# nyasyamorina/font-renderer

Measured on AMD Instinct MI355X. Metric: Mpixel/s AA glyph coverage, higher is better.
Workload: dtype f32

## Files before the change

font-renderer_amd/csrc/fr_c4.hpp:

```cpp
#pragma once
#include "fr_records.hpp"
#include "fr_wave.hpp"

namespace fr {

#ifndef FR_C4_WAVES
#define FR_C4_WAVES 4
#endif
#ifndef FR_C4_OCC
#define FR_C4_OCC 4
#endif
#ifndef FR_C4_PCAP
#define FR_C4_PCAP 448
#endif
#ifndef FR_C4_OCC_SMALL
#define FR_C4_OCC_SMALL 6
#endif
#ifndef FR_DYN_BANDS
#define FR_DYN_BANDS 1
#endif
#ifndef FR_W1_OCC_SMALL
#define FR_W1_OCC_SMALL 6
#endif
enum { C4_WAVES = FR_C4_WAVES, C4_PCAP = FR_C4_PCAP };
// ... 7 lines not shown
    const uint2 a = reinterpret_cast<const uint2 *>(p)[0], b = reinterpret_cast<const uint2 *>(p)[1];
    return make_uint4(a.x, a.y, b.x, b.y);
}
template <uint32_t LSTRIDE>
__device__ __forceinline__ void c4_st16(uint16_t *p, uint4 v)
{
    if ((LSTRIDE * 2) % 16 == 0) { *reinterpret_cast<uint4 *>(p) = v; return; }
    reinterpret_cast<uint2 *>(p)[0] = make_uint2(v.x, v.y);
    reinterpret_cast<uint2 *>(p)[1] = make_uint2(v.z, v.w);
}

struct __attribute__((aligned(8))) Rec40 {
    float a;
    float b;
    float c1, c2;
    float ax, bx, p0x;
    float rden;
    float sgn;
    uint32_t fr;
};

__device__ __forceinline__ uint32_t c4_sel(unsigned long long m, uint32_t if_set, uint32_t if_clear)
{
    uint32_t r;
    asm("v_cndmask_b32_e64 %0, %1, %2, %3" : "=v"(r) : "v"(if_clear), "v"(if_set), "s"(m));
    return r;
}
__device__ __forceinline__ float c4_self(unsigned long long m, float if_set, float if_clear)
{
    return __builtin_bit_cast(float, c4_sel(m, __builtin_bit_cast(uint32_t, if_set), __builtin_bit_cast(uint32_t, if_clear)));
}
__device__ __forceinline__ void c4_store16(void *dst, uint4 v)
{
    typedef uint32_t u32x4 __attribute__((ext_vector_type(4)));
    typedef u32x4 u32x4_u __attribute__((aligned(4)));
    u32x4 w = {v.x, v.y, v.z, v.w};
    __builtin_nontemporal_store(w, reinterpret_cast<u32x4_u *>(dst));
}

template <int FILL = 0>
__device__ __forceinline__ Rec40 c4_make_rec40(const Rec &r, uint32_t ra, uint32_t re)
{
    Rec40 m;
    const bool lin = (int32_t)r.flags < 0;
    m.a = lin ? r.c1 : r.a;
    m.b = r.b; m.c1 = lin ? 0.0f : r.c1; m.c2 = r.c2;
    m.ax = r.ax; m.bx = r.bx; m.p0x = r.p0x; m.rden = r.rden;
    m.sgn = r.sqsign ? -1.0f : 1.0f;
    const uint32_t cb = (lin || FILL) ? (r.flags & 2u) : 2u, zb = (lin || FILL) ? cb : 0u;
    m.fr = ra | (re << 12) | (cb << 24) | (zb << 26) | (lin ? 0x80000000u : 0u);
    return m;
}

template <uint32_t RCAP, int N, uint32_t NCOL, int FILL>
__device__ __forceinline__ uint32_t c4_setup_small(const RenderArgs &A, const Job &job, uint32_t seg0, uint32_t nseg, uint32_t x0s,
                                                   int phase, float *s_cxp, Rec40 *s_rec, uint32_t *s_wcnt, uint32_t *s_tmp, const float *cyt = nullptr)
{
    const uint32_t tid = threadIdx.x, lane = tid & 63u, wave = tid >> 6;
    const uint32_t Hs = job.h * (uint32_t)N;
    RowGeom geo;
    geo.max_y = job.max_y; geo.scale = job.scale; geo.rows = Hs; geo.n = N; geo.phase = phase; geo.cyt = cyt;
    const bool have = lane < 2u * nseg;
    Rec r;
    RowGuess g;
    Piece pc;
    g.empty = true; g.ra = 1u; g.re = 0u;
    uint32_t cls = 3u;
    if (have) {
        record_prep<FILL>(A.seg_pts + 6u * (size_t)(seg0 + (lane >> 1)), lane & 1u, geo, r, g, &pc);
        if (!g.empty) {
            const uint32_t row = (wave == 0u) ? g.ra - 1u : (wave == 1u) ? g.ra : (wave == 2u) ? g.re - 1u : g.re;
            if (row < Hs && (wave != 2u || g.re > g.ra)) cls = (uint32_t)row_class<FILL>(r, pc, geo.cy(row));
        }
    }
    s_tmp[tid] = cls;
    const int32_t min_xs = job.min_x + (int32_t)x0s;
    for (uint32_t j = tid; j < NCOL; j += 256u)
        s_cxp[1u + j] = ((float)(min_xs + (int32_t)(j / (uint32_t)N)) + sub_off((int)(j % (uint32_t)N), N, phase)) / job.scale;
    if (tid == 2) s_cxp[0] = -__builtin_inff();
    if (tid == 3) s_cxp[1u + NCOL] = __builtin_inff();
    __syncthreads();
    if (wave == 0u) {
        Rec40 mine;
        mine.fr = 0u;
        bool live = false;
        if (have) {
            uint32_t ra = g.ra, re = g.re;
            if (!g.empty) {
                const uint32_t c0 = s_tmp[lane], c1 = s_tmp[64u + lane], c2 = s_tmp[128u + lane], c3 = s_tmp[192u + lane];
                const bool ok = (c0 >= 2u) && (c1 <= 1u || c1 == 3u) && re >= ra && (c2 >= 1u) && (c3 == 0u || c3 == 3u);
                if (!ok) record_settle<FILL>(r, geo, ra, re, &pc);
            }
            live = ra < re;
            mine = c4_make_rec40<FILL>(r, ra, re);
        }
        const bool linr = live && (int32_t)mine.fr < 0;
        const unsigned long long lm = __ballot(live && !linr), ll = __ballot(linr), below = (1ull << lane) - 1ull;
        const uint32_t n_quad = (uint32_t)__popcll(lm);
        uint32_t pos = RCAP;
        if ((lm >> lane) & 1ull) pos = (uint32_t)__popcll(lm & below);
        if ((ll >> lane) & 1ull) pos = n_quad + (uint32_t)__popcll(ll & below);
        if (pos < RCAP) s_rec[pos] = mine;
        if (lane == 0u) s_wcnt[0] = min(n_quad + (uint32_t)__popcll(ll), RCAP);
    }
    __syncthreads();
    return s_wcnt[0];
}

template <uint32_t RCAP, int N, uint32_t NCOL, int FILL>
__device__ __forceinline__ uint32_t c4_setup_mid(const RenderArgs &A, const Job &job, uint32_t seg0, uint32_t nseg, uint32_t x0s,
                                                 int phase, float *s_cxp, Rec40 *s_rec, uint32_t *s_wcnt, uint32_t *s_tmp, const float *cyt = nullptr)
{
    const uint32_t tid = threadIdx.x, lane = tid & 63u, wave = tid >> 6;
    const uint32_t c = tid & 127u, h = tid >> 7;
    const uint32_t Hs = job.h * (uint32_t)N;
    RowGeom geo;
    geo.max_y = job.max_y; geo.scale = job.scale; geo.rows = Hs; geo.n = N; geo.phase = phase; geo.cyt = cyt;
    const bool have = c < 2u * nseg;
    Rec r;
    RowGuess g;
    Piece pc;
    g.empty = true; g.ra = 1u; g.re = 0u;
    uint32_t cls0 = 3u, cls1 = 3u;
    if (have) {
        record_prep<FILL>(A.seg_pts + 6u * (size_t)(seg0 + (c >> 1)), c & 1u, geo, r, g, &pc);
        if (!g.empty) {
            const uint32_t end = h ? g.re : g.ra;
            if (end - 1u < Hs && (h == 0u || g.re > g.ra)) cls0 = (uint32_t)row_class<FILL>(r, pc, geo.cy(end - 1u));
            if (end < Hs) cls1 = (uint32_t)row_class<FILL>(r, pc, geo.cy(end));
        }
    }
    s_tmp[tid] = cls0 | (cls1 << 8);
    const int32_t min_xs = job.min_x + (int32_t)x0s;
    for (uint32_t j = tid; j < NCOL; j += 256u)
        s_cxp[1u + j] = ((float)(min_xs + (int32_t)(j / (uint32_t)N)) + sub_off((int)(j % (uint32_t)N), N, phase)) / job.scale;
    if (tid == 2) s_cxp[0] = -__builtin_inff();
    if (tid == 3) s_cxp[1u + NCOL] = __builtin_inff();
    __syncthreads();
    Rec40 mine;
    mine.fr = 0u;
    bool live = false;
    if (h == 0u && have) {
        uint32_t ra = g.ra, re = g.re;
        if (!g.empty) {
            const uint32_t up = s_tmp[c], dn = s_tmp[128u + c];
            const uint32_t c0 = up & 0xffu, c1 = up >> 8, c2 = dn & 0xffu, c3 = dn >> 8;
            const bool ok = (c0 >= 2u) && (c1 <= 1u || c1 == 3u) && re >= ra && (c2 >= 1u) && (c3 == 0u || c3 == 3u);
            if (!ok) record_settle<FILL>(r, geo, ra, re, &pc);
        }
        live = ra < re;
        mine = c4_make_rec40<FILL>(r, ra, re);
    }
    const bool linr = live && (int32_t)mine.fr < 0;
    const unsigned long long lm = __ballot(live && !linr), ll = __ballot(linr), below = (1ull << lane) - 1ull;
    if (lane == 0u && wave < 2u) { s_wcnt[wave] = (uint32_t)__popcll(lm); s_wcnt[2u + wave] = (uint32_t)__popcll(ll); }
    __syncthreads();
    const uint32_t q0 = s_wcnt[0], q1 = s_wcnt[1], l0 = s_wcnt[2], l1 = s_wcnt[3];
    const uint32_t n_quad = q0 + q1;
    uint32_t pos = RCAP;
    if ((lm >> lane) & 1ull) pos = (wave ? q0 : 0u) + (uint32_t)__popcll(lm & below);
    if ((ll >> lane) & 1ull) pos = n_quad + (wave ? l0 : 0u) + (uint32_t)__popcll(ll & below);
    if (wave < 2u && pos < RCAP) s_rec[pos] = mine;
    __syncthreads();
    return min(n_quad + l0 + l1, RCAP);
}

template <uint32_t NW, uint32_t RCAP, int N, uint32_t NCOL, int FILL = 0>
__device__ __forceinline__ uint32_t c4_setup(const RenderArgs &A, const Job &job, uint32_t seg0, uint32_t nseg, uint32_t x0s,
                                             int phase, float *s_cxp, Rec40 *s_rec, uint32_t *s_wcnt, uint32_t *s_tmp, const float *cyt = nullptr)
{
    if (NW == 4u && 2u * nseg <= 64u)
        return c4_setup_small<RCAP, N, NCOL, FILL>(A, job, seg0, nseg, x0s, phase, s_cxp, s_rec, s_wcnt, s_tmp, cyt);
    if (NW == 4u && 2u * nseg <= 128u)
        return c4_setup_mid<RCAP, N, NCOL, FILL>(A, job, seg0, nseg, x0s, phase, s_cxp, s_rec, s_wcnt, s_tmp, cyt);
    const uint32_t tid = threadIdx.x, lane = tid & 63u, wave = tid >> 6;
    const uint32_t Hs = job.h * (uint32_t)N;
    constexpr uint32_t CPT = (RCAP >= 1024u ? 1536u : (RCAP >= 512u ? 768u : 512u)) / (64u * NW);
    s_wcnt = s_tmp;
    Rec40 mine[CPT];
    unsigned long long lm[CPT], ll[CPT];
#pragma unroll
    for (uint32_t it = 0; it < CPT; ++it) {
        const uint32_t c = tid + it * 64u * NW;
        bool live = false;
        lm[it] = 0ull; ll[it] = 0ull;
        mine[it].fr = 0u;
        if (it > 0 && it * 64u * NW >= 2u * nseg) continue;
        if (c < 2u * nseg) {
            Rec r;
            RowGeom geo;
            geo.max_y = job.max_y; geo.scale = job.scale; geo.rows = Hs; geo.n = N; geo.phase = phase; geo.cyt = cyt;
            build_record_rows<FILL>(A.seg_pts + 6u * (size_t)(seg0 + (c >> 1)), c & 1u, geo, r);
            const uint32_t ra = __builtin_bit_cast(uint32_t, r.lo), re = __builtin_bit_cast(uint32_t, r.hi);
            live = ra < re;
            mine[it] = c4_make_rec40<FILL>(r, ra, re);
        }
        const bool linr = live && (int32_t)mine[it].fr < 0;
        lm[it] = __ballot(live && !linr);
        ll[it] = __ballot(linr);
        if (lane == 0) { s_wcnt[it * NW + wave] = (uint32_t)__popcll(lm[it]); s_wcnt[CPT * NW + it * NW + wave] = (uint32_t)__popcll(ll[it]); }
    }
    const int32_t min_xs = job.min_x + (int32_t)x0s;
    for (uint32_t j = tid; j < NCOL; j += 64u * NW)
        s_cxp[1u + j] = ((float)(min_xs + (int32_t)(j / (uint32_t)N)) + sub_off((int)(j % (uint32_t)N), N, phase)) / job.scale;
    if (tid == 2) s_cxp[0] = -__builtin_inff();
    if (tid == 3) s_cxp[1u + NCOL] = __builtin_inff();
    __syncthreads();
    uint32_t rec_cnt = 0;
    {
        uint32_t base_q[CPT], base_l[CPT], n_quad = 0;
#pragma unroll
        for (uint32_t it = 0; it < CPT; ++it) base_q[it] = base_l[it] = 0;
#pragma unroll
        for (uint32_t q = 0; q < CPT * NW; ++q) {
            if (q >= NW && q / NW * 64u * NW >= 2u * nseg) continue;
            const uint32_t cq = s_wcnt[q], cl = s_wcnt[CPT * NW + q];
#pragma unroll
            for (uint32_t it = 0; it < CPT; ++it) {
                base_q[it] += (q < it * NW + wave) ? cq : 0u;
                base_l[it] += (q < it * NW + wave) ? cl : 0u;
            }
            n_quad += cq;
            rec_cnt += cq + cl;
        }
#pragma unroll
        for (uint32_t it = 0; it < CPT; ++it) {
            const unsigned long long below = (1ull << lane) - 1ull;
            uint32_t pos = RCAP;
            if ((lm[it] >> lane) & 1ull) pos = base_q[it] + (uint32_t)__popcll(lm[it] & below);
            if ((ll[it] >> lane) & 1ull) pos = n_quad + base_l[it] + (uint32_t)__popcll(ll[it] & below);
            if (pos < RCAP) s_rec[pos] = mine[it];
        }
    }
    rec_cnt = min(rec_cnt, RCAP);
    __syncthreads();
    return rec_cnt;
}

}
```

font-renderer_amd/csrc/fr_cov4_kernel.inc:

```
    using L = C4Lds<WLOG, RPL, NS, CAP>;
    constexpr uint32_t LSTRIDE = L::LSTRIDE;
    static_assert(NS == 4 || NS == 2, "samples per axis");
    constexpr uint32_t RCAP = L::RCAP;
    constexpr uint32_t NW = C4_WAVES;
    constexpr uint32_t SW = 16u << WLOG;
    constexpr uint32_t NCOL = SW * (uint32_t)NS;
    constexpr uint32_t NWIN = 1u << WLOG;
    constexpr uint32_t PRB = L::PRB;
    constexpr int LN = (NS == 4) ? 2 : 1;
    constexpr bool SPLIT = RPL >= 8 && CAP == 32;
    extern __shared__ __align__(16) unsigned char smem[];

    const uint32_t tid = threadIdx.x, lane = tid & 63u;
    const uint32_t wave = (uint32_t)__builtin_amdgcn_readfirstlane((int)(tid >> 6));
    uint32_t bid = blockIdx.x, strip = 0, bgrp = 0;
    if (A.strips != 1u) { strip = bid % A.strips; bid /= A.strips; }
    if (A.band_groups != 1u) { bgrp = bid % A.band_groups; bid /= A.band_groups; }
    const uint32_t jidx = bid;
    C4_ABL_LAUNCH_ONLY();
    const Job job = A.jobs[jidx];
    const uint32_t x0s = strip * SW;
    const uint32_t band_first = bgrp * A.bands_per_wg;
    if (band_first * PRB >= job.h || x0s >= job.w) return;
    const uint32_t band_end = min(band_first + A.bands_per_wg, (job.h + PRB - 1u) / PRB);
    const uint32_t wlim = min(SW, job.w - x0s);
    const int phase = A.phase_center;
    const uint32_t seg0 = A.job_seg[2u * (size_t)jidx], nseg = A.job_seg[2u * (size_t)jidx + 1u];
    C4_ABL_JOB_ONLY();
    C4_ABL_SEGLOAD_ONLY();
    float *s_cxp = reinterpret_cast<float *>(smem);
    Rec40 *s_rec = reinterpret_cast<Rec40 *>(smem + L::CX);
    unsigned char *wregion = smem + L::OFF_WAVES + (size_t)wave * L::WAVE;
    uint32_t *s_wcnt = reinterpret_cast<uint32_t *>(smem + L::OFF_WCNT);

    uint32_t *const s_next_band = s_wcnt + 15;
    if (tid == 0u) *s_next_band = band_first + NW;
    const uint32_t rec_cnt = c4_setup<NW, RCAP, NS, NCOL, FILL>(A, job, seg0, nseg, x0s, phase, s_cxp, s_rec, s_wcnt, reinterpret_cast<uint32_t *>(smem + L::OFF_WAVES));
    const int32_t min_xs = job.min_x + (int32_t)x0s;
    const float jscale = job.scale * (float)NS;
    const float joff = (float)min_xs * (float)NS + (phase ? 0.5f : 0.0f) - 1.0f;
    const float ncolf = (float)NCOL;
    const bool few = RPL == 2 || rec_cnt <= 128u;
    const uint32_t per = few ? 2u : (uint32_t)RPL;
    uint32_t rra[RPL], rre[RPL];
#pragma unroll
    for (int i = 0; i < RPL; ++i) {
        const uint32_t k = per * lane + (uint32_t)i;
        const bool have = k < rec_cnt && (!few || i < 2);
        const uint32_t f = s_rec[have ? k : 0u].fr;
        rra[i] = have ? (f & 0xfffu) : 1u;
        rre[i] = have ? ((f >> 12) & 0xfffu) : 0u;
    }

    uint16_t *s_lists = reinterpret_cast<uint16_t *>(wregion);
    uint16_t *s_pairs = reinterpret_cast<uint16_t *>(wregion + L::OFF_PAIRS);
    float *s_cy = reinterpret_cast<float *>(wregion + L::OFF_CY);
    uint32_t *s_cnt = reinterpret_cast<uint32_t *>(wregion + L::OFF_CNT);
    int16_t *s_roff = reinterpret_cast<int16_t *>(wregion + L::OFF_ROFF);
    unsigned char *s_E = wregion;

    C4_ABL_SETUP_ONLY();
#if FR_DYN_BANDS
    for (uint32_t band = band_first + wave; band < band_end;
         band = (uint32_t)__builtin_amdgcn_readfirstlane((int)(lane == 0u ? atomicAdd(s_next_band, 1u) : 0u))) {
#else
    for (uint32_t band0 = band_first; band0 < band_end; band0 += NW) {
        const uint32_t band = band0 + wave;
        if (band >= band_end) break;
#endif
        const uint32_t y0 = band * PRB;
        const uint32_t row_b0 = band * 64u;
        const float cy = ((float)(job.max_y - (int32_t)(y0 + (lane >> LN))) - sub_off((int)(lane & (uint32_t)(NS - 1)), NS, phase)) / job.scale;
        uint16_t *mylist = s_lists + lane * LSTRIDE;
        auto init_lists = [&]() {
            const uint4 ones = make_uint4(0xfffdfffdu, 0xfffdfffdu, 0xfffdfffdu, 0xfffdfffdu);
#pragma unroll
            for (uint32_t q = 0; q < CAP / 8u; ++q) c4_st16<LSTRIDE>(mylist + 8u * q, ones);
            s_cnt[lane] = 0u;
        };
        init_lists();
        s_cy[lane] = cy;

        uint32_t c[RPL], off0 = 0u, tot;
        {
            uint32_t r0[RPL], csum = 0;
            {
                const uint32_t lo = row_b0, hi = row_b0 + 64u;
#pragma unroll
                for (int i = 0; i < RPL; ++i) {
                    r0[i] = max(rra[i], lo);
                    const uint32_t r1 = min(rre[i], hi);
                    c[i] = r1 > r0[i] ? r1 - r0[i] : 0u;
                    csum += c[i];
                }
            }
            const uint32_t incl = wave_incl_add(csum);
            tot = (uint32_t)__builtin_amdgcn_readlane((int)incl, 63);
            if (tot) {
                off0 = incl - csum;
                {
                    uint32_t off = off0, ro[RPL];
#pragma unroll
                    for (int i = 0; i < RPL; ++i) {
                        ro[i] = (r0[i] - row_b0 - off) & 0xffffu;
                        off += c[i];
                    }
                    if (few) *reinterpret_cast<uint32_t *>(s_roff + 2u * lane) = ro[0] | (ro[1] << 16);
                    else if constexpr (RPL == 4) *reinterpret_cast<uint2 *>(s_roff + 4u * lane) = make_uint2(ro[0] | (ro[1] << 16), ro[2] | (ro[3] << 16));
                    else if constexpr (RPL >= 8) {
#pragma unroll
                    for (int q8 = 0; q8 < RPL / 8; ++q8)
                        reinterpret_cast<uint4 *>(s_roff + (uint32_t)RPL * lane)[q8] = make_uint4(ro[8 * q8] | (ro[8 * q8 + 1] << 16), ro[8 * q8 + 2] | (ro[8 * q8 + 3] << 16),
                                                                                                  ro[8 * q8 + 4] | (ro[8 * q8 + 5] << 16), ro[8 * q8 + 6] | (ro[8 * q8 + 7] << 16));
                }
                }
            }
        }
        auto eval_pass = [&](uint32_t jlo, uint32_t jspan) {
            (void)jlo; (void)jspan;
            if (tot) {
                const uint32_t npairs = tot;
                uint32_t carry = 0u;
              for (uint32_t base = 0; base < npairs; base += (uint32_t)C4_PCAP) {
                if (C4_PCAP >= 512 || lane < C4_PCAP / 8) reinterpret_cast<uint4 *>(s_pairs)[lane] = make_uint4(0, 0, 0, 0);
                wave_lds_sync();
                {
                    uint32_t off = off0 - base;
#pragma unroll
                    for (int i = 0; i < RPL; ++i) {
                        if (c[i] && off < (uint32_t)C4_PCAP) s_pairs[off] = (uint16_t)(per * lane + (uint32_t)i + 1u);
                        off += c[i];
                    }
                }
                wave_lds_sync();
                const uint32_t nhere = min(npairs - base, (uint32_t)C4_PCAP);
                uint32_t k_cur = max(wave_incl_max((uint32_t)s_pairs[lane]), carry);
                carry = (uint32_t)__builtin_amdgcn_readlane((int)k_cur, 63);
                for (uint32_t p0 = 0; p0 < nhere && C4_ABL_KEEP(3); p0 += 64u) {
                    const uint32_t pn = min(p0 + 64u + lane, (uint32_t)C4_PCAP - 1u);
                    const uint32_t s_next = wave_incl_max((uint32_t)s_pairs[pn]);
                    {
                        const uint32_t p = base + p0 + lane, k1 = k_cur;
                        const bool livep = p < npairs;
#if C4_ABL_NODECODE
                        const uint32_t row = (p + (k1 & 1u)) & 63u;
                        const uint32_t raddr = L::CX + ((lane & 3u) + (A.n_jobs == 0xffffffffu ? k1 : 0u)) * (uint32_t)sizeof(Rec40);
#else
                        const uint32_t row = (uint32_t)((int32_t)p + (int32_t)s_roff[k1 - 1u]);
                        const uint32_t raddr = __umul24(k1, (uint32_t)sizeof(Rec40)) + (L::CX - (uint32_t)sizeof(Rec40));
#endif
                        const Rec40 r = *reinterpret_cast<const Rec40 *>(smem + raddr);
                        const float cyr = s_cy[row & 63u];
                        const unsigned long long linm = __builtin_amdgcn_sicmp((int32_t)r.fr, 0, 40 );
                        auto body = [&](auto kind) {
                            constexpr int KIND = decltype(kind)::value;
                            float num;
                            if (KIND == 2) {
                                num = cyr - r.b;
                            } else {
                                const float delta0 = cyr * r.a + r.c1 - r.c2;
                                const float delta = FILL ? __builtin_fmaxf(delta0, 0.0f) : delta0;
                                const float sq = sqrt_rn(delta);
                                const float numq = r.b + sq * r.sgn;
                                num = (KIND == 1) ? numq : c4_self(linm, cyr - r.b, numq);
                            }
                            const float t = div_by_int(num, r.a, r.rden);
                            const float xx = (r.ax * t + r.bx) * t + r.p0x;
                            uint32_t code;
                            if (KIND == 2) {
                                code = (r.fr >> 24) & 3u;
                            } else {
                                const float dy = r.a * t - r.b;
                                if (KIND == 1) code = FILL ? ((r.fr >> 24) & 3u) : ((dy > 0.0f) ? 0u : 2u);
                                else code = (dy > 0.0f) ? ((r.fr >> 26) & 3u) : ((r.fr >> 24) & 3u);
                            }
                            const float gf = __builtin_amdgcn_fmed3f(__builtin_fmaf(xx, jscale, -joff), 0.0f, ncolf);
                            int J = (int)gf;
                            {
                                const float c0 = s_cxp[J], c1 = s_cxp[J + 1];
                                const bool good = (c0 <= xx) & (xx < c1);
                                if (__builtin_expect(!good & livep, 0)) {
                                    while (s_cxp[J + 1] <= xx) ++J;
                                    while (s_cxp[J] > xx) --J;
                                }
                            }
                            bool keep = livep & (J > 0);
                            if constexpr (SPLIT) keep = livep & ((uint32_t)(J - 1) - jlo < jspan);
                            if (keep) {
                                const uint32_t pos = atomicAdd(&s_cnt[row & 63u], 1u);
                                uint16_t *rowlist = s_lists + __umul24(row & 63u, LSTRIDE);
                                rowlist[min(pos, (uint32_t)CAP)] = (uint16_t)(((uint32_t)J << 2) | code);
                            }
                        };
                        body(std::integral_constant<int, 0>{});
                    }
                    k_cur = max(s_next, carry);
                    carry = (uint32_t)__builtin_amdgcn_readlane((int)k_cur, 63);
                }
                wave_lds_sync();
              }
            }
        };
        eval_pass(0u, NCOL);
        C4_ABL_EVAL_ONLY();
        uint32_t cnt = s_cnt[lane];
        uint8_t *const out_band = reinterpret_cast<uint8_t *>(A.out) + ((size_t)job.out_y + y0) * A.out_stride + job.out_x + x0s;
        const uint32_t wx = lane & (NWIN - 1u);
        const uint32_t hlim = min(PRB, job.h - y0);
                const bool edge = __builtin_amdgcn_readfirstlane((int)((wlim < SW) | (hlim < PRB))) != 0;
        if (__ballot(cnt != 0u) == 0ull) {
            for (uint32_t yl = lane >> WLOG; yl < PRB; yl += (64u >> WLOG)) {
                const uint4 z = make_uint4(0, 0, 0, 0);
                unsigned char *dst = out_band + (size_t)yl * A.out_stride + 16u * wx;
                if (!edge) c4_store16(dst, z);
                else c4_store_clip(dst, z, yl < hlim ? (int)wlim - (int)(16u * wx) : 0);
            }
            wave_lds_sync();
            continue;
        }
        auto pull_sort = [&](uint32_t (&dd)[16], uint32_t n, bool blank, uint32_t &H, uint32_t &mx) {
#pragma unroll
            for (int q = 0; q < 4; ++q) {
                uint4 v = make_uint4(0xfffdfffdu, 0xfffdfffdu, 0xfffdfffdu, 0xfffdfffdu);
                if (q < CAP / 8 && (q == 0 || __ballot(n > (uint32_t)(8 * q)) != 0ull)) v = c4_ld16<LSTRIDE>(mylist + 8 * q);
                dd[4 * q + 0] = v.x; dd[4 * q + 1] = v.y; dd[4 * q + 2] = v.z; dd[4 * q + 3] = v.w;
            }
            if (__ballot(blank)) {
#pragma unroll
                for (int q = 0; q < 16; ++q) dd[q] = blank ? 0xfffdfffdu : dd[q];
            }
            if (CAP > 16 && __ballot(n > 16u && !blank) != 0ull) {
                packed_sort<16>(dd); H = 16u;
                mx = __ballot(n > 28u) ? 32u : (__ballot(n > 24u) ? 28u : (__ballot(n > 20u) ? 24u : 20u));
            } else if (CAP > 8 && __ballot(n > 8u && !blank) != 0ull) {
                packed_sort<8>(dd); H = 8u;
                mx = __ballot(n > 12u) ? 16u : 12u;
            } else {
                packed_sort<4>(dd); H = 4u;
                mx = __ballot(n > 4u) ? 8u : 4u;
            }
        };
        bool ovf = cnt > (uint32_t)CAP;
        uint32_t d[16];
// ... 286 lines not shown
```

font-renderer_amd/csrc/fr_device.hpp:

```cpp
#pragma once
#include <hip/hip_runtime.h>
#include <stdint.h>

#pragma clang fp contract(off)

namespace fr {

struct __attribute__((aligned(16))) Rec {
    float lo, hi, a, b, c1, c2, ax, bx, p0x;
    uint32_t flags;
    float rden;
    uint32_t sqsign;
};

__device__ __forceinline__ float div_by_int(float x, float d, float rd)
{
    const float q = x * rd;
    const float r = __builtin_fmaf(-q, d, x);
    return __builtin_fmaf(r, rd, q);
}
__device__ __forceinline__ float sqrt_rn(float x)
{
    const float s = __builtin_amdgcn_sqrtf(x);
    const float sm = __builtin_bit_cast(float, __builtin_bit_cast(int, s) - 1);
    const float sp = __builtin_bit_cast(float, __builtin_bit_cast(int, s) + 1);
    const float rm = __builtin_fmaf(-sm, s, x);
    const float rp = __builtin_fmaf(-sp, s, x);
    float r = (rm <= 0.0f) ? sm : s;
    r = (rp > 0.0f) ? sp : r;
    return r;
}
enum : uint32_t {
    REC_LINEAR = 0x80000000u,
    REC_NEG_ROOT = 2u,
    REC_LIN_MINUS = 4u,
    REC_LIN_PLUS = 2u
};

struct Job {
    uint32_t glyph;
    int32_t min_x, max_y;
    uint32_t w, h;
    uint32_t out_x, out_y;
    float scale;
};

struct RenderArgs {
    const Job *jobs;
    const uint32_t *glyph_seg_start;
    const uint32_t *job_seg;
    const uint32_t *glyph_rec_count;
    const Rec *recs;
    const int16_t *pts;
    const uint32_t *seg_p0;
    const int16_t *seg_pts;
    const uint32_t *job_bits;
    const uint32_t *bits;
    uint32_t fused;
    uint32_t uniform;
    void *out;
    uint64_t out_stride;
    uint32_t n_jobs, bands, strips, strip_w, kmax;
    uint32_t bands_per_wg, band_groups;
    int32_t phase_center;
    uint32_t lds_pad;
    uint32_t nwin_log, lds_region, lds_rec_bytes, lds_wave_bytes, lds_tail;
};

template <typename K>
inline hipError_t launch_kernel(K *kern, dim3 grid, dim3 block, size_t lds, hipStream_t stream, const RenderArgs &a)
{
    if (lds > 48 * 1024) {
        const hipError_t e = hipFuncSetAttribute(reinterpret_cast<const void *>(kern), hipFuncAttributeMaxDynamicSharedMemorySize, (int)lds);
        if (e != hipSuccess) return e;
    }
    hipLaunchKernelGGL(kern, grid, block, lds, stream, a);
    return hipGetLastError();
}

__host__ __device__ inline uint32_t f2key(float f)
{
    uint32_t b;
    __builtin_memcpy(&b, &f, 4);
// ... 74 lines not shown
```

font-renderer_amd/csrc/fr_records.hpp:

```cpp
#pragma once
#include "fr_device.hpp"

namespace fr {

__device__ __forceinline__ int classify(const Rec &r, float cy)
{
    if (r.flags & REC_LINEAR) {
        float t = rec_t_lin(r, cy);
        bool up = r.c1 > 0.0f;
        if (t < 0.0f) return up ? 0 : 2;
        if (t >= 1.0f) return up ? 2 : 0;
        return 1;
    }
    float delta = cy * r.a + r.c1 - r.c2;
    if (delta < 0.0f) return (r.a > 0.0f) ? 0 : 2;
    float t = rec_t_quad(r, cy);
    bool neg = (r.flags & REC_NEG_ROOT) != 0;
    if (t < 0.0f) return neg ? 2 : 0;
    if (t >= 1.0f) return neg ? 0 : 2;
    return 1;
}

__device__ __noinline__ uint32_t first_at_least(float ra, float rb, float rc1, float rc2, uint32_t rflags, int T, uint32_t L, uint32_t H)
{
// ... 39 lines not shown
    }
    auto probe3 = [&](float c) {
        const float d = fmaxf(4.0f * w, fabsf(c) * 4.76837158e-07f);
        probe(c - d);
        probe(c);
        probe(c + d);
    };
    probe3(p0y);
    probe3(p2y);
    if (quad) probe3(vert);
    if (LB >= HB) return false;
    if (LB == kmin) LB = first_at_least(r.a, r.b, r.c1, r.c2, r.flags, 1, kmin, HB);
    if (HB == kmax + 1u) HB = first_at_least(r.a, r.b, r.c1, r.c2, r.flags, 2, LB, kmax + 1u);
    if (LB >= HB) return false;
    (void)seen1;
    lo = key2f(LB);
    hi = key2f(HB - 1u);
    return true;
}


__device__ inline bool build_record(const int16_t *p, uint32_t root, Rec &r)
{
    const float p0x = (float)p[0], p0y = (float)p[1];
    const float p1x = (float)p[2], p1y = (float)p[3];
    const float p2x = (float)p[4], p2y = (float)p[5];
    const float a = p0y - 2 * p1y + p2y;
    r.ax = p0x - 2 * p1x + p2x;
    r.bx = 2 * (p1x - p0x);
    r.p0x = p0x;
    r.sqsign = root ? 0x80000000u : 0u;
    if (a == 0.0f) {
        if (root != 0u || p2y == p0y) return false;
        r.a = 0.0f; r.b = p0y; r.c1 = p2y - p0y; r.c2 = 0.0f;
        r.rden = 1.0f / r.c1;
        r.flags = REC_LINEAR | ((p0y < p2y) ? REC_LIN_MINUS : REC_LIN_PLUS);
    } else {
        r.a = a; r.b = p0y - p1y; r.c1 = p1y * p1y; r.c2 = p0y * p2y;
        r.rden = 1.0f / a;
        r.flags = root ? REC_NEG_ROOT : 0u;
    }
    float lo, hi;
    if (!accept_bracket(r, p0y, p2y, lo, hi)) return false;
    r.lo = lo; r.hi = hi;
    return true;
}

struct RowGeom {
    int32_t max_y;
    float scale;
    uint32_t rows;
    int n, phase;
    const float *cyt = nullptr;
    __device__ __forceinline__ float cy(uint32_t r) const
    {
        if (cyt) return cyt[r];
        return ((float)(max_y - (int32_t)(r / (uint32_t)n)) - sub_off((int)(r % (uint32_t)n), n, phase)) / scale;
    }
    __device__ __forceinline__ float row_of(float c) const
    {
        return ((float)max_y - c * scale) * (float)n - (phase ? 0.5f : 0.0f);
    }
};

__device__ __forceinline__ int classify_row(const Rec &r, float cy)
{
    const bool lin = (r.flags & REC_LINEAR) != 0;
    const float delta = cy * r.a + r.c1 - r.c2;
    const float sq = sqrt_rn(delta);
    const float num = lin ? (cy - r.b) : ((r.flags & REC_NEG_ROOT) ? (r.b - sq) : (r.b + sq));
    const float t = div_by_int(num, lin ? r.c1 : r.a, r.rden);
    const bool falls = lin ? !(r.c1 > 0.0f) : ((r.flags & REC_NEG_ROOT) != 0);
    int cl = 1;
    if (t >= 1.0f) cl = falls ? 0 : 2;
    if (t < 0.0f) cl = falls ? 2 : 0;
    if (!lin && delta < 0.0f) cl = (r.a > 0.0f) ? 0 : 2;
    return cl;
}

struct Piece {
    float ylo, yhi;
    float a;
    double cv;
    uint32_t vend;
};
__device__ __forceinline__ bool fill_at_or_above_vertex(const Piece &pc, float cy)
{
    const double d = __builtin_fma((double)pc.a, (double)cy, pc.cv);
    return pc.a > 0.0f ? d >= 0.0 : d <= 0.0;
}
__device__ __forceinline__ int classify_fill(const Piece &pc, float cy)
{
    const bool above = (pc.vend == 2u) ? fill_at_or_above_vertex(pc, cy) : (cy >= pc.yhi);
    const bool below = (pc.vend == 1u) ? !fill_at_or_above_vertex(pc, cy) : (cy < pc.ylo);
    return above ? 2 : (below ? 0 : 1);
}
template <int FILL>
__device__ __forceinline__ int row_class(const Rec &r, const Piece &pc, float cy)
{
    if constexpr (FILL != 0) return classify_fill(pc, cy);
    else return classify_row(r, cy);
}

struct RowGuess {
    uint32_t ra, re;
    bool empty;
};

template <int FILL = 0>
__device__ __forceinline__ void record_prep(const int16_t *p, uint32_t root, const RowGeom &G, Rec &r, RowGuess &g, Piece *pc = nullptr)
// ... 126 lines not shown
```

font-renderer_amd/csrc/fr_selftest.hip:

```cpp
#include "../../include/fr_raster.h"
#include "fr_device.hpp"

namespace fr {

__global__ __launch_bounds__(256) void selftest_div_kernel(uint32_t d_lo, uint32_t n_d,
                                                           unsigned long long *mismatches,
                                                           uint32_t *first_bad)
{
    const uint32_t d_idx = blockIdx.x / 32u, part = blockIdx.x % 32u;
    if (d_idx >= n_d) return;
    const float d = (float)(d_lo + d_idx);
    const float rd = 1.0f / d, rdn = 1.0f / (-d);
    uint32_t bad = 0, bad_x = 0;
    for (uint32_t m = part * 256u + threadIdx.x; m < (1u << 23); m += 32u * 256u) {
        const float x = __uint_as_float(0x3f800000u | m);
        const float xs = __uint_as_float(0x2f800000u | m);
        const float xl = __uint_as_float(0x4f800000u | m);
        const bool ok = (__float_as_uint(div_by_int(x, d, rd)) == __float_as_uint(x / d)) &&
                        (__float_as_uint(div_by_int(x, -d, rdn)) == __float_as_uint(x / -d)) &&
                        (__float_as_uint(div_by_int(-xs, d, rd)) == __float_as_uint(-xs / d)) &&
                        (__float_as_uint(div_by_int(xl, d, rd)) == __float_as_uint(xl / d));
        if (!ok) { ++bad; bad_x = 0x3f800000u | m; }
    }
    if (bad) {
        atomicAdd(mismatches, (unsigned long long)bad);
        atomicMax(&first_bad[0], d_lo + d_idx);
        first_bad[1] = bad_x;
    }
}

__global__ __launch_bounds__(256) void selftest_sqrt_kernel(uint32_t e_lo, unsigned long long *mismatches, uint32_t *first_bad)
{
    const uint32_t e = e_lo + blockIdx.x / 32u, part = blockIdx.x % 32u;
    uint32_t bad = 0, bad_x = 0;
    for (uint32_t m = part * 256u + threadIdx.x; m < (1u << 23); m += 32u * 256u) {
        const uint32_t bits = (e << 23) | m;
        const float x = __uint_as_float(bits);
        if (__float_as_uint(sqrt_rn(x)) != __float_as_uint(__builtin_sqrtf(x))) { ++bad; bad_x = bits; }
    }
    if (bad) {
        atomicAdd(mismatches, (unsigned long long)bad);
        first_bad[0] = bad_x;
    }
}

}

extern "C" int fr_selftest_sqrt(uint64_t *mismatches, uint32_t *bad_x_bits)
{
    if (!mismatches) return FR_E_INVALID;
    unsigned long long *d_m = nullptr;
    uint32_t *d_b = nullptr;
    if (hipMalloc(&d_m, 8) != hipSuccess || hipMalloc(&d_b, 8) != hipSuccess) return FR_E_HIP;
    (void)hipMemset(d_m, 0, 8);
    (void)hipMemset(d_b, 0, 8);
    const uint32_t e_lo = 97u, e_hi = 192u;
    hipLaunchKernelGGL(fr::selftest_sqrt_kernel, dim3((e_hi - e_lo + 1u) * 32u), dim3(256), 0, 0, e_lo, d_m, d_b);
    unsigned long long m = 0;
    uint32_t b = 0;
    hipError_t e = hipMemcpy(&m, d_m, 8, hipMemcpyDeviceToHost);
    if (e == hipSuccess) e = hipMemcpy(&b, d_b, 4, hipMemcpyDeviceToHost);
    (void)hipFree(d_m);
    (void)hipFree(d_b);
    if (e != hipSuccess) return FR_E_HIP;
    *mismatches = m;
    if (bad_x_bits) *bad_x_bits = b;
    return FR_OK;
}

extern "C" int fr_selftest_division(uint32_t d_lo, uint32_t d_hi, uint64_t *mismatches,
                                    uint32_t *bad_divisor, uint32_t *bad_x_bits)
{
    if (!mismatches || d_lo < 1 || d_hi < d_lo || d_hi > (1u << 17)) return FR_E_INVALID;
    unsigned long long *d_m = nullptr;
    uint32_t *d_b = nullptr;
    if (hipMalloc(&d_m, 8) != hipSuccess || hipMalloc(&d_b, 8) != hipSuccess) return FR_E_HIP;
    (void)hipMemset(d_m, 0, 8);
    (void)hipMemset(d_b, 0, 8);
    const uint32_t n_d = d_hi - d_lo + 1;
    for (uint32_t off = 0; off < n_d; off += 4096u) {
        const uint32_t n = n_d - off < 4096u ? n_d - off : 4096u;
        hipLaunchKernelGGL(fr::selftest_div_kernel, dim3(n * 32u), dim3(256), 0, 0, d_lo + off, n, d_m, d_b);
    }
    unsigned long long m = 0;
    uint32_t b[2] = {0, 0};
    hipError_t e = hipMemcpy(&m, d_m, 8, hipMemcpyDeviceToHost);
    if (e == hipSuccess) e = hipMemcpy(b, d_b, 8, hipMemcpyDeviceToHost);
    (void)hipFree(d_m);
    (void)hipFree(d_b);
    if (e != hipSuccess) return FR_E_HIP;
    *mismatches = m;
    if (bad_divisor) *bad_divisor = b[0];
    if (bad_x_bits) *bad_x_bits = b[1];
    return FR_OK;
}
```

font-renderer_amd/csrc/fr_win1_kernel.inc:

```
    using L = W1Lds<WLOG, RPL>;
    constexpr uint32_t NW = C4_WAVES;
    constexpr uint32_t RCAP = L::RCAP;
    constexpr uint32_t NCOL = L::NCOL;
    constexpr uint32_t NWIN = 1u << WLOG;
    constexpr uint32_t PCAP = L::PCAP;
    constexpr uint32_t ESZ = (MODE == MODE1_WINDING_I16) ? 2u : 1u;
    extern __shared__ __align__(16) unsigned char smem[];

    const uint32_t tid = threadIdx.x, lane = tid & 63u;
    const uint32_t wave = (WLOG == 4 && RPL == 2) ? (tid >> 6) : (uint32_t)__builtin_amdgcn_readfirstlane((int)(tid >> 6));
    uint32_t bid = blockIdx.x, strip = 0, bgrp = 0;
    if (A.strips != 1u) { strip = bid % A.strips; bid /= A.strips; }
    if (A.band_groups != 1u) { bgrp = bid % A.band_groups; bid /= A.band_groups; }
    const uint32_t jidx = bid;
    const Job job = A.jobs[jidx];
    const uint32_t x0s = strip * NCOL;
    const uint32_t band_first = bgrp * A.bands_per_wg;
    if (band_first * W1_ROWS >= job.h || x0s >= job.w) return;
    const uint32_t band_end = min(band_first + A.bands_per_wg, (job.h + W1_ROWS - 1u) / W1_ROWS);
    const uint32_t wlim = min(NCOL, job.w - x0s);
    const int phase = A.phase_center;
    const uint32_t seg0 = A.job_seg[2u * (size_t)jidx], nseg = A.job_seg[2u * (size_t)jidx + 1u];

    float *s_cxp = reinterpret_cast<float *>(smem);
    Rec40 *s_rec = reinterpret_cast<Rec40 *>(smem + L::CX);
    unsigned char *wregion = smem + L::OFF_WAVES + (size_t)wave * L::WAVE;
    uint32_t *s_wcnt = reinterpret_cast<uint32_t *>(smem + L::OFF_WCNT);

    const float soff = phase ? 0.5f : 0.0f;
    const float *cyt = nullptr;
    if (job.h <= 256u) {
        float *t = reinterpret_cast<float *>(smem + L::OFF_CYT);
        if (tid < job.h) t[tid] = ((float)(job.max_y - (int32_t)tid) - soff) / job.scale;
        __syncthreads();
        cyt = t;
    }
    const uint32_t rec_cnt_v = c4_setup<NW, RCAP, 1, NCOL, FILL>(A, job, seg0, nseg, x0s, phase, s_cxp, s_rec, s_wcnt, reinterpret_cast<uint32_t *>(smem + L::OFF_WAVES), cyt);
    const uint32_t rec_cnt = (WLOG == 4 && RPL == 2) ? rec_cnt_v : (uint32_t)__builtin_amdgcn_readfirstlane((int)rec_cnt_v);
    const int32_t min_xs = job.min_x + (int32_t)x0s;
    const float jscale = job.scale;
    const float joff = (float)min_xs + soff - 1.0f;
    const float ncolf = (float)NCOL;
    const bool few = RPL == 2 || rec_cnt <= 128u;
    const uint32_t per = few ? 2u : (uint32_t)RPL;
    uint32_t rra[RPL], rre[RPL];
#pragma unroll
    for (int i = 0; i < RPL; ++i) {
        const uint32_t k = per * lane + (uint32_t)i;
        const bool have = k < rec_cnt && (!few || i < 2);
        const uint32_t f = s_rec[have ? k : 0u].fr;
        rra[i] = have ? (f & 0xfffu) : 1u;
        rre[i] = have ? ((f >> 12) & 0xfffu) : 0u;
    }

    unsigned char *s_E = wregion;
    uint16_t *s_pairs = reinterpret_cast<uint16_t *>(wregion + L::OFF_PAIRS);
    float *s_cy = reinterpret_cast<float *>(wregion + L::OFF_CY);
    uint32_t *s_cnt = reinterpret_cast<uint32_t *>(wregion + L::OFF_CNT);
    int16_t *s_roff = reinterpret_cast<int16_t *>(wregion + L::OFF_ROFF);
    const uint32_t wx = lane & (NWIN - 1u);

    for (uint32_t band0 = band_first; band0 < band_end; band0 += NW) {
        const uint32_t band = band0 + wave;
        if (band >= band_end) break;
        const uint32_t y0 = band * W1_ROWS;
        const float cy = cyt ? cyt[y0 + (lane & 15u)] : ((float)(job.max_y - (int32_t)(y0 + (lane & 15u))) - soff) / job.scale;
        {
            uint4 *z = reinterpret_cast<uint4 *>(s_E);
            const uint4 bias = make_uint4(0x20202020u, 0x20202020u, 0x20202020u, 0x20202020u);
            constexpr uint32_t NZ = L::E / 16u;
#pragma unroll
            for (uint32_t q = 0; q < (NZ + 63u) / 64u; ++q)
                if (NZ % 64u == 0u || lane + 64u * q < NZ) z[lane + 64u * q] = bias;
        }
        if (lane < 16u) { s_cy[lane] = cy; s_cnt[lane] = 0u; }

        uint32_t rr0 = 0;
        while (rr0 < W1_ROWS) {
            uint32_t span = W1_ROWS - rr0;
            uint32_t c[RPL], r0[RPL], csum, incl, tot;
            for (;;) {
                const uint32_t lo = y0 + rr0, hi = lo + span;
                csum = 0;
#pragma unroll
                for (int i = 0; i < RPL; ++i) {
                    r0[i] = max(rra[i], lo);
                    const uint32_t r1 = min(rre[i], hi);
                    c[i] = r1 > r0[i] ? r1 - r0[i] : 0u;
                    csum += c[i];
                }
                incl = wave_incl_add(csum);
                tot = (uint32_t)__builtin_amdgcn_readlane((int)incl, 63);
                if (tot <= PCAP || span == 1u) break;
                span >>= 1;
            }
            if (tot) {
#pragma unroll
                for (uint32_t q = 0; q < (PCAP / 8u + 63u) / 64u; ++q)
                    if (PCAP / 8u % 64u == 0u || lane + 64u * q < PCAP / 8u) reinterpret_cast<uint4 *>(s_pairs)[lane + 64u * q] = make_uint4(0, 0, 0, 0);
                wave_lds_sync();
                uint32_t off = incl - csum;
                uint32_t ro[RPL];
#pragma unroll
                for (int i = 0; i < RPL; ++i) {
                    if (c[i]) s_pairs[off] = (uint16_t)(per * lane + (uint32_t)i + 1u);
                    ro[i] = (r0[i] - y0 - off) & 0xffffu;
                    off += c[i];
                }
                if (few) *reinterpret_cast<uint32_t *>(s_roff + 2u * lane) = ro[0] | (ro[1] << 16);
                else if constexpr (RPL == 4) *reinterpret_cast<uint2 *>(s_roff + 4u * lane) = make_uint2(ro[0] | (ro[1] << 16), ro[2] | (ro[3] << 16));
                else if constexpr (RPL >= 8) {
#pragma unroll
                    for (int q8 = 0; q8 < RPL / 8; ++q8)
                        reinterpret_cast<uint4 *>(s_roff + (uint32_t)RPL * lane)[q8] = make_uint4(ro[8 * q8] | (ro[8 * q8 + 1] << 16), ro[8 * q8 + 2] | (ro[8 * q8 + 3] << 16),
                                                                                                  ro[8 * q8 + 4] | (ro[8 * q8 + 5] << 16), ro[8 * q8 + 6] | (ro[8 * q8 + 7] << 16));
                }
                wave_lds_sync();
                const uint32_t npairs = tot;
                uint32_t k_cur = wave_incl_max((uint32_t)s_pairs[lane]);
// ... 292 lines not shown
```

Baseline: 2.485 million.

## Use exact reciprocal multiply for power-of-two scales and pre-scaled LDS addressing

Adds a ScaleDiv helper that replaces the division by job.scale with a multiply by an exact reciprocal when the scale is a power of two, and applies it across setup, row-geometry and window kernels. Separately, the cov4 pair-decode loop is changed to keep row offsets and record indices pre-scaled as byte offsets from a per-wave base register, so LDS addresses are formed with fewer integer ops. It also adds a sqrt_fast routine with a selftest kernel that is not yet used on the hot path. These aim to cut ALU work in setup and pair decoding, at the cost of more intricate address arithmetic and a forced VGPR for the wave base.

```diff
diff --git a/font-renderer_amd/csrc/fr_c4.hpp b/font-renderer_amd/csrc/fr_c4.hpp
--- a/font-renderer_amd/csrc/fr_c4.hpp
+++ b/font-renderer_amd/csrc/fr_c4.hpp
@@ -83,14 +83,26 @@
     return m;
 }
 
+template <int N, uint32_t NCOL, uint32_t STEP>
+__device__ __forceinline__ void c4_fill_cx(float *s_cxp, uint32_t tid, int32_t min_xs, int phase, const ScaleDiv &sdiv)
+{
+    auto num = [&](uint32_t j) { return (float)(min_xs + (int32_t)(j / (uint32_t)N)) + sub_off((int)(j % (uint32_t)N), N, phase); };
+    if (sdiv.pow2) {
+        for (uint32_t j = tid; j < NCOL; j += STEP) s_cxp[1u + j] = num(j) * sdiv.inv;
+    } else {
+        for (uint32_t j = tid; j < NCOL; j += STEP) s_cxp[1u + j] = num(j) / sdiv.scale;
+    }
+}
+
 template <uint32_t RCAP, int N, uint32_t NCOL, int FILL>
 __device__ __forceinline__ uint32_t c4_setup_small(const RenderArgs &A, const Job &job, uint32_t seg0, uint32_t nseg, uint32_t x0s,
                                                    int phase, float *s_cxp, Rec40 *s_rec, uint32_t *s_wcnt, uint32_t *s_tmp, const float *cyt = nullptr)
 {
     const uint32_t tid = threadIdx.x, lane = tid & 63u, wave = tid >> 6;
     const uint32_t Hs = job.h * (uint32_t)N;
+    const ScaleDiv sdiv = scale_div(job.scale);
     RowGeom geo;
-    geo.max_y = job.max_y; geo.scale = job.scale; geo.rows = Hs; geo.n = N; geo.phase = phase; geo.cyt = cyt;
+    geo.max_y = job.max_y; geo.set_scale(sdiv); geo.rows = Hs; geo.n = N; geo.phase = phase; geo.cyt = cyt;
     const bool have = lane < 2u * nseg;
     Rec r;
     RowGuess g;
@@ -106,8 +118,7 @@
     }
     s_tmp[tid] = cls;
     const int32_t min_xs = job.min_x + (int32_t)x0s;
-    for (uint32_t j = tid; j < NCOL; j += 256u)
-        s_cxp[1u + j] = ((float)(min_xs + (int32_t)(j / (uint32_t)N)) + sub_off((int)(j % (uint32_t)N), N, phase)) / job.scale;
+    c4_fill_cx<N, NCOL, 256u>(s_cxp, tid, min_xs, phase, sdiv);
     if (tid == 2) s_cxp[0] = -__builtin_inff();
     if (tid == 3) s_cxp[1u + NCOL] = __builtin_inff();
     __syncthreads();
@@ -145,8 +156,9 @@
     const uint32_t tid = threadIdx.x, lane = tid & 63u, wave = tid >> 6;
     const uint32_t c = tid & 127u, h = tid >> 7;
     const uint32_t Hs = job.h * (uint32_t)N;
+    const ScaleDiv sdiv = scale_div(job.scale);
     RowGeom geo;
-    geo.max_y = job.max_y; geo.scale = job.scale; geo.rows = Hs; geo.n = N; geo.phase = phase; geo.cyt = cyt;
+    geo.max_y = job.max_y; geo.set_scale(sdiv); geo.rows = Hs; geo.n = N; geo.phase = phase; geo.cyt = cyt;
     const bool have = c < 2u * nseg;
     Rec r;
     RowGuess g;
@@ -163,8 +175,7 @@
     }
     s_tmp[tid] = cls0 | (cls1 << 8);
     const int32_t min_xs = job.min_x + (int32_t)x0s;
-    for (uint32_t j = tid; j < NCOL; j += 256u)
-        s_cxp[1u + j] = ((float)(min_xs + (int32_t)(j / (uint32_t)N)) + sub_off((int)(j % (uint32_t)N), N, phase)) / job.scale;
+    c4_fill_cx<N, NCOL, 256u>(s_cxp, tid, min_xs, phase, sdiv);
     if (tid == 2) s_cxp[0] = -__builtin_inff();
     if (tid == 3) s_cxp[1u + NCOL] = __builtin_inff();
     __syncthreads();
@@ -206,6 +217,7 @@
         return c4_setup_mid<RCAP, N, NCOL, FILL>(A, job, seg0, nseg, x0s, phase, s_cxp, s_rec, s_wcnt, s_tmp, cyt);
     const uint32_t tid = threadIdx.x, lane = tid & 63u, wave = tid >> 6;
     const uint32_t Hs = job.h * (uint32_t)N;
+    const ScaleDiv sdiv = scale_div(job.scale);
     constexpr uint32_t CPT = (RCAP >= 1024u ? 1536u : (RCAP >= 512u ? 768u : 512u)) / (64u * NW);
     s_wcnt = s_tmp;
     Rec40 mine[CPT];
@@ -220,7 +232,7 @@
         if (c < 2u * nseg) {
             Rec r;
             RowGeom geo;
-            geo.max_y = job.max_y; geo.scale = job.scale; geo.rows = Hs; geo.n = N; geo.phase = phase; geo.cyt = cyt;
+            geo.max_y = job.max_y; geo.set_scale(sdiv); geo.rows = Hs; geo.n = N; geo.phase = phase; geo.cyt = cyt;
             build_record_rows<FILL>(A.seg_pts + 6u * (size_t)(seg0 + (c >> 1)), c & 1u, geo, r);
             const uint32_t ra = __builtin_bit_cast(uint32_t, r.lo), re = __builtin_bit_cast(uint32_t, r.hi);
             live = ra < re;
@@ -232,8 +244,7 @@
         if (lane == 0) { s_wcnt[it * NW + wave] = (uint32_t)__popcll(lm[it]); s_wcnt[CPT * NW + it * NW + wave] = (uint32_t)__popcll(ll[it]); }
     }
     const int32_t min_xs = job.min_x + (int32_t)x0s;
-    for (uint32_t j = tid; j < NCOL; j += 64u * NW)
-        s_cxp[1u + j] = ((float)(min_xs + (int32_t)(j / (uint32_t)N)) + sub_off((int)(j % (uint32_t)N), N, phase)) / job.scale;
+    c4_fill_cx<N, NCOL, 64u * NW>(s_cxp, tid, min_xs, phase, sdiv);
     if (tid == 2) s_cxp[0] = -__builtin_inff();
     if (tid == 3) s_cxp[1u + NCOL] = __builtin_inff();
     __syncthreads();
diff --git a/font-renderer_amd/csrc/fr_cov4_kernel.inc b/font-renderer_amd/csrc/fr_cov4_kernel.inc
--- a/font-renderer_amd/csrc/fr_cov4_kernel.inc
+++ b/font-renderer_amd/csrc/fr_cov4_kernel.inc
@@ -37,6 +37,7 @@
     if (tid == 0u) *s_next_band = band_first + NW;
     const uint32_t rec_cnt = c4_setup<NW, RCAP, NS, NCOL, FILL>(A, job, seg0, nseg, x0s, phase, s_cxp, s_rec, s_wcnt, reinterpret_cast<uint32_t *>(smem + L::OFF_WAVES));
     const int32_t min_xs = job.min_x + (int32_t)x0s;
+    const ScaleDiv sdiv = scale_div(job.scale);
     const float jscale = job.scale * (float)NS;
     const float joff = (float)min_xs * (float)NS + (phase ? 0.5f : 0.0f) - 1.0f;
     const float ncolf = (float)NCOL;
@@ -58,6 +59,12 @@
     uint32_t *s_cnt = reinterpret_cast<uint32_t *>(wregion + L::OFF_CNT);
     int16_t *s_roff = reinterpret_cast<int16_t *>(wregion + L::OFF_ROFF);
     unsigned char *s_E = wregion;
+    constexpr bool VBASE = c4_occ(CAP, WLOG, RPL) <= 4 && RPL != 8;
+    uint32_t wreg = L::OFF_WAVES + wave * L::WAVE;
+    if constexpr (VBASE) asm volatile("" : "+v"(wreg));
+    const uint32_t lane4 = lane << 2;
+    const uint32_t mk0 = 2u * (per * lane + 1u);
+    static_assert(LSTRIDE % 2u == 0u && C4_PCAP % 64 == 0, "row lists are whole dwords; chunks are whole trips");
 
     C4_ABL_SETUP_ONLY();
 #if FR_DYN_BANDS
@@ -70,7 +77,7 @@
 #endif
         const uint32_t y0 = band * PRB;
         const uint32_t row_b0 = band * 64u;
-        const float cy = ((float)(job.max_y - (int32_t)(y0 + (lane >> LN))) - sub_off((int)(lane & (uint32_t)(NS - 1)), NS, phase)) / job.scale;
+        const float cy = sdiv((float)(job.max_y - (int32_t)(y0 + (lane >> LN))) - sub_off((int)(lane & (uint32_t)(NS - 1)), NS, phase));
         uint16_t *mylist = s_lists + lane * LSTRIDE;
         auto init_lists = [&]() {
             const uint4 ones = make_uint4(0xfffdfffdu, 0xfffdfffdu, 0xfffdfffdu, 0xfffdfffdu);
@@ -102,7 +109,7 @@
                     uint32_t off = off0, ro[RPL];
 #pragma unroll
                     for (int i = 0; i < RPL; ++i) {
-                        ro[i] = (r0[i] - row_b0 - off) & 0xffffu;
+                        ro[i] = ((r0[i] - row_b0 - off) & 63u) << 2;
                         off += c[i];
                     }
                     if (few) *reinterpret_cast<uint32_t *>(s_roff + 2u * lane) = ro[0] | (ro[1] << 16);
@@ -128,7 +135,7 @@
                     uint32_t off = off0 - base;
 #pragma unroll
                     for (int i = 0; i < RPL; ++i) {
-                        if (c[i] && off < (uint32_t)C4_PCAP) s_pairs[off] = (uint16_t)(per * lane + (uint32_t)i + 1u);
+                        if (c[i] && off < (uint32_t)C4_PCAP) s_pairs[off] = (uint16_t)(mk0 + 2u * (uint32_t)i);
                         off += c[i];
                     }
                 }
@@ -136,21 +143,24 @@
                 const uint32_t nhere = min(npairs - base, (uint32_t)C4_PCAP);
                 uint32_t k_cur = max(wave_incl_max((uint32_t)s_pairs[lane]), carry);
                 carry = (uint32_t)__builtin_amdgcn_readlane((int)k_cur, 63);
+                uint32_t pn2 = 2u * lane + 128u;
                 for (uint32_t p0 = 0; p0 < nhere && C4_ABL_KEEP(3); p0 += 64u) {
-                    const uint32_t pn = min(p0 + 64u + lane, (uint32_t)C4_PCAP - 1u);
-                    const uint32_t s_next = wave_incl_max((uint32_t)s_pairs[pn]);
+                    const uint32_t s_next = wave_incl_max((uint32_t)*reinterpret_cast<const uint16_t *>(smem + (wreg + min(pn2, 2u * (uint32_t)C4_PCAP - 2u)) + L::OFF_PAIRS));
+                    pn2 += 128u;
                     {
-                        const uint32_t p = base + p0 + lane, k1 = k_cur;
-                        const bool livep = p < npairs;
+                        const uint32_t k2 = k_cur;
+                        const bool livep = lane < npairs - base - p0;
 #if C4_ABL_NODECODE
-                        const uint32_t row = (p + (k1 & 1u)) & 63u;
-                        const uint32_t raddr = L::CX + ((lane & 3u) + (A.n_jobs == 0xffffffffu ? k1 : 0u)) * (uint32_t)sizeof(Rec40);
+                        const uint32_t row4 = (lane4 + ((k2 & 2u) << 1)) & 252u;
+                        const uint32_t raddr = L::CX + ((lane & 3u) + (A.n_jobs == 0xffffffffu ? (k2 >> 1) : 0u)) * (uint32_t)sizeof(Rec40);
 #else
-                        const uint32_t row = (uint32_t)((int32_t)p + (int32_t)s_roff[k1 - 1u]);
-                        const uint32_t raddr = __umul24(k1, (uint32_t)sizeof(Rec40)) + (L::CX - (uint32_t)sizeof(Rec40));
+                        const uint32_t roff4 = *reinterpret_cast<const uint16_t *>(smem + (wreg + k2) + (L::OFF_ROFF - 2u));
+                        const uint32_t row4 = (lane4 + roff4) & 252u;
+                        const uint32_t raddr = __umul24(k2, (uint32_t)sizeof(Rec40) / 2u) + (L::CX - (uint32_t)sizeof(Rec40));
 #endif
-                        const Rec40 r = *reinterpret_cast<const Rec40 *>(smem + raddr);
-                        const float cyr = s_cy[row & 63u];
+                        const Rec40 r = *reinterpret_cast<const Rec40 *>(__builtin_assume_aligned(smem + raddr, 8));
+                        const uint32_t rowa = wreg + row4;
+                        const float cyr = *reinterpret_cast<const float *>(smem + rowa + L::OFF_CY);
                         const unsigned long long linm = __builtin_amdgcn_sicmp((int32_t)r.fr, 0, 40 );
                         auto body = [&](auto kind) {
                             constexpr int KIND = decltype(kind)::value;
@@ -187,8 +197,8 @@
                             bool keep = livep & (J > 0);
                             if constexpr (SPLIT) keep = livep & ((uint32_t)(J - 1) - jlo < jspan);
                             if (keep) {
-                                const uint32_t pos = atomicAdd(&s_cnt[row & 63u], 1u);
-                                uint16_t *rowlist = s_lists + __umul24(row & 63u, LSTRIDE);
+                                const uint32_t pos = atomicAdd(reinterpret_cast<uint32_t *>(smem + rowa + L::OFF_CNT), 1u);
+                                uint16_t *rowlist = reinterpret_cast<uint16_t *>(smem + (wreg + __umul24(row4, LSTRIDE / 2u)));
                                 rowlist[min(pos, (uint32_t)CAP)] = (uint16_t)(((uint32_t)J << 2) | code);
                             }
                         };
diff --git a/font-renderer_amd/csrc/fr_device.hpp b/font-renderer_amd/csrc/fr_device.hpp
--- a/font-renderer_amd/csrc/fr_device.hpp
+++ b/font-renderer_amd/csrc/fr_device.hpp
@@ -29,6 +29,34 @@
     float r = (rm <= 0.0f) ? sm : s;
     r = (rp > 0.0f) ? sp : r;
     return r;
+}
+template <int VARIANT>
+__device__ __forceinline__ float sqrt_fast(float x)
+{
+    const float s = __builtin_amdgcn_sqrtf(x);
+    const float g = VARIANT == 0 ? __builtin_amdgcn_rcpf(s) : __builtin_amdgcn_rsqf(x);
+    const float h = __builtin_fminf(0.5f * g, 1.0e+30f);
+    const float r = __builtin_fmaf(-s, s, x);
+    return __builtin_fmaf(r, h, s);
+}
+struct ScaleDiv {
+    float scale = 1.0f, inv = 1.0f;
+    bool pow2 = false;
+    __device__ __forceinline__ float operator()(float x) const
+    {
+        if (pow2) return x * inv;
+        return x / scale;
+    }
+};
+__device__ __forceinline__ ScaleDiv scale_div(float scale)
+{
+    ScaleDiv d;
+    const uint32_t b = (uint32_t)__builtin_amdgcn_readfirstlane(__builtin_bit_cast(int, scale));
+    const uint32_t e = (b >> 23) & 0xffu;
+    d.scale = scale;
+    d.pow2 = (b & 0x007fffffu) == 0u && e - 107u <= 40u;
+    d.inv = __builtin_bit_cast(float, (b & 0x80000000u) | ((254u - e) << 23));
+    return d;
 }
 enum : uint32_t {
     REC_LINEAR = 0x80000000u,
diff --git a/font-renderer_amd/csrc/fr_records.hpp b/font-renderer_amd/csrc/fr_records.hpp
--- a/font-renderer_amd/csrc/fr_records.hpp
+++ b/font-renderer_amd/csrc/fr_records.hpp
@@ -115,10 +115,15 @@
     uint32_t rows;
     int n, phase;
     const float *cyt = nullptr;
+    float inv = 1.0f;
+    bool pow2 = false;
+    __device__ __forceinline__ void set_scale(const ScaleDiv &d) { scale = d.scale; inv = d.inv; pow2 = d.pow2; }
     __device__ __forceinline__ float cy(uint32_t r) const
     {
         if (cyt) return cyt[r];
-        return ((float)(max_y - (int32_t)(r / (uint32_t)n)) - sub_off((int)(r % (uint32_t)n), n, phase)) / scale;
+        const float num = (float)(max_y - (int32_t)(r / (uint32_t)n)) - sub_off((int)(r % (uint32_t)n), n, phase);
+        if (pow2) return num * inv;
+        return num / scale;
     }
     __device__ __forceinline__ float row_of(float c) const
     {
diff --git a/font-renderer_amd/csrc/fr_selftest.hip b/font-renderer_amd/csrc/fr_selftest.hip
--- a/font-renderer_amd/csrc/fr_selftest.hip
+++ b/font-renderer_amd/csrc/fr_selftest.hip
@@ -44,6 +44,53 @@
     }
 }
 
+template <int VARIANT>
+__global__ __launch_bounds__(256) void selftest_sqrt_fast_kernel(uint32_t e_lo, unsigned long long *mismatches, uint32_t *first_bad)
+{
+    const uint32_t e = e_lo + blockIdx.x / 32u, part = blockIdx.x % 32u;
+    uint32_t bad = 0, bad_x = 0;
+    for (uint32_t m = part * 256u + threadIdx.x; m < (1u << 23); m += 32u * 256u) {
+        const uint32_t bits = (e << 23) | m;
+        const float x = __uint_as_float(bits);
+        if (__float_as_uint(sqrt_fast<VARIANT>(x)) != __float_as_uint(__builtin_sqrtf(x))) { ++bad; bad_x = bits; }
+    }
+    if (blockIdx.x == 0u && threadIdx.x == 0u) {
+        float z = 0.0f, n = -2.0f;
+        asm volatile("" : "+v"(z), "+v"(n));
+        if (__float_as_uint(sqrt_fast<VARIANT>(z)) != 0u) { ++bad; bad_x = 0u; }
+        const float sn = sqrt_fast<VARIANT>(n);
+        if (sn == sn) { ++bad; bad_x = __float_as_uint(n); }
+    }
+    if (bad) {
+        atomicAdd(mismatches, (unsigned long long)bad);
+        first_bad[0] = bad_x;
+    }
+}
+
+}
+
+extern "C" int fr_selftest_sqrt_fast(int variant, uint64_t *mismatches, uint32_t *bad_x_bits)
+{
+    if (!mismatches || variant < 0 || variant > 1) return FR_E_INVALID;
+    unsigned long long *d_m = nullptr;
+    uint32_t *d_b = nullptr;
+    if (hipMalloc(&d_m, 8) != hipSuccess || hipMalloc(&d_b, 8) != hipSuccess) return FR_E_HIP;
+    (void)hipMemset(d_m, 0, 8);
+    (void)hipMemset(d_b, 0, 8);
+    const uint32_t e_lo = 97u, e_hi = 192u;
+    const dim3 grid((e_hi - e_lo + 1u) * 32u), block(256);
+    if (variant == 0) hipLaunchKernelGGL(fr::selftest_sqrt_fast_kernel<0>, grid, block, 0, 0, e_lo, d_m, d_b);
+    else hipLaunchKernelGGL(fr::selftest_sqrt_fast_kernel<1>, grid, block, 0, 0, e_lo, d_m, d_b);
+    unsigned long long m = 0;
+    uint32_t b = 0;
+    hipError_t e = hipMemcpy(&m, d_m, 8, hipMemcpyDeviceToHost);
+    if (e == hipSuccess) e = hipMemcpy(&b, d_b, 4, hipMemcpyDeviceToHost);
+    (void)hipFree(d_m);
+    (void)hipFree(d_b);
+    if (e != hipSuccess) return FR_E_HIP;
+    *mismatches = m;
+    if (bad_x_bits) *bad_x_bits = b;
+    return FR_OK;
 }
 
 extern "C" int fr_selftest_sqrt(uint64_t *mismatches, uint32_t *bad_x_bits)
diff --git a/font-renderer_amd/csrc/fr_win1_kernel.inc b/font-renderer_amd/csrc/fr_win1_kernel.inc
--- a/font-renderer_amd/csrc/fr_win1_kernel.inc
+++ b/font-renderer_amd/csrc/fr_win1_kernel.inc
@@ -28,10 +28,11 @@
     uint32_t *s_wcnt = reinterpret_cast<uint32_t *>(smem + L::OFF_WCNT);
 
     const float soff = phase ? 0.5f : 0.0f;
+    const ScaleDiv sdiv = scale_div(job.scale);
     const float *cyt = nullptr;
     if (job.h <= 256u) {
         float *t = reinterpret_cast<float *>(smem + L::OFF_CYT);
-        if (tid < job.h) t[tid] = ((float)(job.max_y - (int32_t)tid) - soff) / job.scale;
+        if (tid < job.h) t[tid] = sdiv((float)(job.max_y - (int32_t)tid) - soff);
         __syncthreads();
         cyt = t;
     }
@@ -64,7 +65,7 @@
         const uint32_t band = band0 + wave;
         if (band >= band_end) break;
         const uint32_t y0 = band * W1_ROWS;
-        const float cy = cyt ? cyt[y0 + (lane & 15u)] : ((float)(job.max_y - (int32_t)(y0 + (lane & 15u))) - soff) / job.scale;
+        const float cy = cyt ? cyt[y0 + (lane & 15u)] : sdiv((float)(job.max_y - (int32_t)(y0 + (lane & 15u))) - soff);
         {
             uint4 *z = reinterpret_cast<uint4 *>(s_E);
             const uint4 bias = make_uint4(0x20202020u, 0x20202020u, 0x20202020u, 0x20202020u);
```

New measurement: 2.530 million, median of 6. 1.8% higher.
